# lukifer23/Matrix0

Hardware: AMD Instinct MI355X
Metric: self-play games/sec at 800 sims/move, ResNet-24 53M; 1/2/4/8 MI355X (higher is better)
Workload: dtype f16

## Files before the change

matrix0_amd/csrc/attn_block.hip:

```cpp
#include "attn_math.h"
#include "conv_epilogue.h"

typedef float float4v __attribute__((ext_vector_type(4)));

namespace {
constexpr int AB_PIECE = 12288;
constexpr int AB_PIECES_PER_GROUP = 7;
constexpr int AB_GROUPS = 10;
constexpr int AB_X = 0;
constexpr int AB_QK = 81920;
constexpr int AB_VT = AB_QK + 16384;
constexpr int AB_VROW = 68;
constexpr int AB_RING = AB_VT + 4 * 16 * AB_VROW * 2;
constexpr int AB_PAR = AB_RING + 4 * AB_PIECE;
constexpr int AB_LDS = AB_PAR + 4 * 320 * 4;

struct AbLane {
    int tid, lane, w;
    int l15, lq, r31, half;
    int wm, wn;
    size_t b0;
    uint32_t xa[2];
    int wq0, wq1, wpo;
    uint32_t ring_a, of_a;
    const char* wsrc;
    char* ring_w;
    int au, aboard, ahl, aqt, aq;
};
struct AbRegs {
    float4v oc[20];
    float4v qa[2][3];
    half8 fs[2][5];
    half8 of;
    half8 bias8[4];
    half2v visp[16];
};
}

__device__ __forceinline__ void ab_load64(half8& b0, half8& b1, half8& b2, half8& b3, const half8* p) {
    asm volatile("global_load_dwordx4 %0, %4, off\n\tglobal_load_dwordx4 %1, %4, off offset:16\n\t"
                 "global_load_dwordx4 %2, %4, off offset:32\n\tglobal_load_dwordx4 %3, %4, off offset:48"
                 : "=&v"(b0), "=&v"(b1), "=&v"(b2), "=&v"(b3) : "v"(p) : "memory");
}
template <int OFF>
__device__ __forceinline__ void ab_lds16(half8& d, uint32_t addr) {
    asm volatile("ds_read_b128 %0, %1 offset:%2" : "=v"(d) : "v"(addr), "n"(OFF) : "memory");
}
template <int N>
__device__ __forceinline__ void ab_lds_arrived(half8& f0, half8& f1, half8& f2, half8& f3, half8& f4, half8& f5) {
    static_assert(N == 0 || N == 5, "");
    if constexpr (N == 0) asm volatile("s_waitcnt lgkmcnt(0)" : "+v"(f0), "+v"(f1), "+v"(f2), "+v"(f3), "+v"(f4), "+v"(f5) :: "memory");
    else asm volatile("s_waitcnt lgkmcnt(5)" : "+v"(f0), "+v"(f1), "+v"(f2), "+v"(f3), "+v"(f4), "+v"(f5) :: "memory");
}
template <int CTRL>
__device__ __forceinline__ float ab_dpp(float v) {
    return __builtin_bit_cast(float, __builtin_amdgcn_update_dpp(0, __builtin_bit_cast(int, v), CTRL, 0xF, 0xF, true));
}
__device__ __forceinline__ float ab_row_sum(float v) {
    v += ab_dpp<0xB1>(v);
    v += ab_dpp<0x4E>(v);
    v += ab_dpp<0x141>(v);
    v += ab_dpp<0x140>(v);
    return v;
}

#define AB_WAIT(n) asm volatile("s_waitcnt vmcnt(" #n ")" ::: "memory")
#define AB_LGKM0() asm volatile("s_waitcnt lgkmcnt(0)" ::: "memory")

__device__ __forceinline__ char* ab_smem() {
    extern __shared__ __attribute__((aligned(16))) char smem[];
    return smem;
}

__device__ __forceinline__ AbLane ab_lane(const AttnBlockArgs& a) {
    AbLane L;
    L.tid = threadIdx.x; L.lane = L.tid & 63;
    L.w = __builtin_amdgcn_readfirstlane(L.tid >> 6);
    L.l15 = L.lane & 15; L.lq = L.lane >> 4; L.r31 = L.lane & 31; L.half = L.lane >> 5;
    L.wm = L.w >> 1; L.wn = L.w & 1;
    L.b0 = (size_t)blockIdx.x * 2;
    const int l15 = L.l15, lq = L.lq, w = L.w;
    const int xrow0 = 32 * L.wm + l15;
    const int xsw = (xrow0 >> 1) & 7;
    const int xe0 = ((lq ^ xsw) & 7) * 16, xe1 = (((4 + lq) ^ xsw) & 7) * 16;
    const uint32_t lds0 = (uint32_t)(uintptr_t)ab_smem();
    L.xa[0] = lds0 + AB_X + xrow0 * 640 + xe0; L.xa[1] = lds0 + AB_X + xrow0 * 640 + xe1;
    const int wsw = (l15 >> 1) & 7;
    L.wq0 = (3 * L.wn * 16 + l15) * 128 + ((lq ^ wsw) & 7) * 16;
    L.wq1 = (3 * L.wn * 16 + l15) * 128 + (((4 + lq) ^ wsw) & 7) * 16;
    L.wpo = l15 * 64 + ((lq ^ (4 - (l15 >> 2))) & 3) * 16;
    L.ring_a = lds0 + AB_RING;
    L.of_a = lds0 + AB_QK + (lq >> 1) * 4096 + (16 * w + l15) * 32 + ((lq & 1) ^ (l15 >> 3)) * 16;
    L.wsrc = reinterpret_cast<const char*>(a.wpack) + w * 1536 + L.lane * 16;
    L.ring_w = ab_smem() + AB_RING + w * 1536;
    L.au = w >> 1; L.aboard = L.au >> 1; L.ahl = L.au & 1; L.aqt = w & 1;
    L.aq = L.aqt * 32 + L.r31;
    return L;
}

__device__ __forceinline__ void ab_issue(const AbLane& L, int t) {
    const char* s = L.wsrc + (size_t)t * AB_PIECE;
    char* d = L.ring_w + (t & 3) * AB_PIECE;
    glds16(s, d);
    if (L.lane < 32) glds16(s + 1024, d + 1024);
}

__device__ __forceinline__ void ab_prologue(const AttnBlockArgs& a, const AbLane& L) {
    const char* xg = reinterpret_cast<const char*>(a.x) + L.b0 * 64 * 640;
#pragma unroll
    for (int n = 0; n < 10; ++n) {
        const int idx = L.w * 10 + n;
        const int q = idx * 64 + L.lane;
        const int row = q / 40, pos = q - row * 40;
        const int src = (pos & ~7) | ((pos ^ (row >> 1)) & 7);
        glds16(xg + row * 640 + src * 16, ab_smem() + AB_X + idx * 1024);
    }
    ab_issue(L, 0); ab_issue(L, 1); ab_issue(L, 2);
    const int tid = L.tid;
    if (tid < 320) {
        float* par = reinterpret_cast<float*>(ab_smem() + AB_PAR);
        par[tid] = a.ln_g[tid]; par[320 + tid] = a.ln_b[tid];
        par[640 + tid] = a.y2 ? a.gn2_gamma[tid] : 0.f; par[960 + tid] = a.y2 ? a.gn2_beta[tid] : 0.f;
    }
}

__device__ __forceinline__ void ab_visibility(const AttnBlockArgs& a, const AbLane& L, half2v (&visp)[16]) {
    const uint64_t m = a.mask[L.aq];
    static_for<0, 32>([&](auto i_) __attribute__((always_inline)) {
        constexpr int i = decltype(i_)::value;
        constexpr int kt = i >> 4, r = i & 15;
        const int key = kt * 32 + 8 * (r >> 2) + 4 * L.half + (r & 3);
        visp[i >> 1][i & 1] = (_Float16)(float)((m >> key) & 1);
    });
}

__device__ __forceinline__ void ab_zero_qa(float4v (&qa)[2][3]) {
    const float4v zero4 = {0.f, 0.f, 0.f, 0.f};
    static_for<0, 2>([&](auto i_) __attribute__((always_inline)) {
        static_for<0, 3>([&](auto j_) __attribute__((always_inline)) { qa[decltype(i_)::value][decltype(j_)::value] = zero4; });
    });
}

template <bool HP, int U>
__device__ __forceinline__ void ab_load(const AbLane& L, AbRegs& R, const int T) {
    constexpr int S = U & 1, i = U >> 1, kk = U & 1;
    const uint32_t slot = L.ring_a + (uint32_t)(((T + i) & 3) * AB_PIECE);
    if constexpr (HP && i < 2) {
        if constexpr (U == 0) ab_lds16<0>(R.of, L.of_a);
        const uint32_t pa = slot + L.wpo;
        static_for<0, 5>([&](auto jj_) __attribute__((always_inline)) {
            constexpr int jj = decltype(jj_)::value;
            ab_lds16<(5 * kk + jj) * 1024>(R.fs[S][jj], pa);
        });
    } else {
        constexpr int p = i - (HP ? 2 : 0);
        ab_lds16<128 * p>(R.fs[S][3], L.xa[kk]);
        ab_lds16<128 * p + 16 * 640>(R.fs[S][4], L.xa[kk]);
        const uint32_t wa = slot + (kk ? L.wq1 : L.wq0);
        static_for<0, 3>([&](auto j_) __attribute__((always_inline)) {
            constexpr int j = decltype(j_)::value;
            ab_lds16<j * 2048>(R.fs[S][j], wa);
        });
    }
}
template <int U, int N>
__device__ __forceinline__ void ab_arrived(AbRegs& R) {
    constexpr int S = U & 1;
    ab_lds_arrived<N>(R.fs[S][0], R.fs[S][1], R.fs[S][2], R.fs[S][3], R.fs[S][4], R.of);
}
template <bool HP, int U>
__device__ __forceinline__ void ab_mma(AbRegs& R) {
    constexpr int S = U & 1, i = U >> 1, kk = U & 1;
    if constexpr (HP && i < 2) {
        static_for<0, 5>([&](auto jj_) __attribute__((always_inline)) {
            constexpr int c = 10 * i + 5 * kk + decltype(jj_)::value;
            R.oc[c] = __builtin_amdgcn_mfma_f32_16x16x32_f16(R.fs[S][decltype(jj_)::value], R.of, R.oc[c], 0, 0, 0);
        });
    } else {
        static_for<0, 3>([&](auto j_) __attribute__((always_inline)) {
            constexpr int j = decltype(j_)::value;
            R.qa[0][j] = __builtin_amdgcn_mfma_f32_16x16x32_f16(R.fs[S][j], R.fs[S][3], R.qa[0][j], 0, 0, 0);
            R.qa[1][j] = __builtin_amdgcn_mfma_f32_16x16x32_f16(R.fs[S][j], R.fs[S][4], R.qa[1][j], 0, 0, 0);
        });
    }
}

template <bool HP, bool HQ>
__device__ __forceinline__ void ab_sequence(const AttnBlockArgs& a, const AbLane& L, AbRegs& R, const int T, const int g) {
    constexpr int NP = (HP ? 2 : 0) + (HQ ? 5 : 0), NU = 2 * NP;
    constexpr int BU = NU - 3;
    AB_LGKM0();
    AB_WAIT(4);
    __builtin_amdgcn_s_barrier();
    asm volatile("" ::: "memory");
    ab_load<HP, 0>(L, R, T);
    ab_issue(L, T + 3);
    static_for<0, NU>([&](auto u_) __attribute__((always_inline)) {
        constexpr int u = decltype(u_)::value;
        if constexpr (u + 1 < NU) {
            if constexpr (u & 1) {
                ab_arrived<u, 0>(R);
                AB_WAIT(4);
                __builtin_amdgcn_s_barrier();
                asm volatile("" ::: "memory");
            }
            ab_load<HP, u + 1>(L, R, T);
            if constexpr (u & 1) ab_issue(L, T + (u >> 1) + 4);
            else ab_arrived<u, 5>(R);
        } else {
            ab_arrived<u, 0>(R);
        }
        if constexpr (HQ && u == BU) {
            const half8* bp = reinterpret_cast<const half8*>(a.bias) + ((size_t)((2 * g + L.ahl) * 2 + L.aqt) * 64 + L.lane) * 4;
            ab_load64(R.bias8[0], R.bias8[1], R.bias8[2], R.bias8[3], bp);
        }
        ab_mma<HP, u>(R);
        __builtin_amdgcn_sched_barrier(0);
    });
}

__device__ __forceinline__ void ab_stage_qkv(const AbLane& L, const float4v (&qa)[2][3]) {
    char* const smem = ab_smem();
    const int lane = L.lane, l15 = L.l15, lq = L.lq;
    static_for<0, 2>([&](auto i_) __attribute__((always_inline)) {
        static_for<0, 3>([&](auto j_) __attribute__((always_inline)) {
            constexpr int i = decltype(i_)::value, j = decltype(j_)::value;
            const int J = 3 * L.wn + j, type = J >> 1, hl = J & 1;
            const int token = 32 * L.wm + 16 * i + l15;
            const half4v h = {(_Float16)qa[i][j][0], (_Float16)qa[i][j][1], (_Float16)qa[i][j][2], (_Float16)qa[i][j][3]};
            if (type < 2) {
                *reinterpret_cast<half4v*>(smem + AB_QK + type * 8192 + hl * 4096 + token * 32 + (((lq >> 1) ^ (l15 >> 3)) & 1) * 16 + (lq & 1) * 8) = h;
            } else {
                const int unit = (token >> 6) * 2 + hl, sq = token & 63;
                union { half2v h2; uint32_t u; } p01, p23;
                p01.h2 = half2v{h[0], h[1]}; p23.h2 = half2v{h[2], h[3]};
                const bool odd = (lane & 1) != 0;
                const uint32_t own = odd ? p23.u : p01.u;
                const uint32_t recv = (uint32_t)__builtin_amdgcn_update_dpp(0, (int)(odd ? p01.u : p23.u), 0xB1, 0xF, 0xF, true);
                const uint32_t ta = odd ? recv : own, tb = odd ? own : recv;
                const uint32_t w0 = __builtin_amdgcn_perm(tb, ta, 0x05040100u);
                const uint32_t w1 = __builtin_amdgcn_perm(tb, ta, 0x07060302u);
                uint32_t* vt = reinterpret_cast<uint32_t*>(reinterpret_cast<_Float16*>(smem + AB_VT) +
                                                           (unit * 16 + 4 * lq + (odd ? 2 : 0)) * AB_VROW + (sq & ~1));
                vt[0] = w0; vt[AB_VROW / 2] = w1;
            }
        });
    });
    AB_LGKM0();
    __builtin_amdgcn_s_barrier();
    asm volatile("" ::: "memory");
}

__device__ __forceinline__ void ab_attend(const AbLane& L, AbRegs& R, float isd, float clampv, float wm, float wu) {
    const int half = L.half, r31 = L.r31;
    const char* Kb = ab_smem() + AB_QK + 8192 + L.ahl * 4096 + L.aboard * 64 * 32;
    const int hsw = 16 * (half ^ ((r31 >> 3) & 1));
    const half8 kf0 = *reinterpret_cast<const half8*>(Kb + r31 * 32 + hsw);
    const half8 kf1 = *reinterpret_cast<const half8*>(Kb + (32 + r31) * 32 + hsw);
    char* Qp = ab_smem() + AB_QK + L.ahl * 4096 + (L.aboard * 64 + L.aq) * 32 + hsw;
    const half8 qfr = *reinterpret_cast<const half8*>(Qp);
    half8 vf[2][2];
    attn_v_frags(reinterpret_cast<const _Float16*>(ab_smem() + AB_VT) + (L.au * 16 + L.l15) * AB_VROW, half, vf);
    float16v st[2];
    attn_scores(kf0, kf1, qfr, st);
    asm volatile("s_waitcnt vmcnt(0)" : "+v"(R.bias8[0]), "+v"(R.bias8[1]), "+v"(R.bias8[2]), "+v"(R.bias8[3]) :: "memory");
    auto bias = [&](auto kt_, auto g_) __attribute__((always_inline)) {
        constexpr int bi = decltype(kt_)::value * 16 + 4 * decltype(g_)::value;
        const half8 b = R.bias8[bi >> 3];
        return half4v{b[bi & 7], b[(bi & 7) + 1], b[(bi & 7) + 2], b[(bi & 7) + 3]};
    };
    auto vis = [&](auto kt_, auto g_) __attribute__((always_inline)) {
        constexpr int bi = decltype(kt_)::value * 16 + 4 * decltype(g_)::value;
        return half4v{R.visp[bi >> 1][0], R.visp[bi >> 1][1], R.visp[(bi >> 1) + 1][0], R.visp[(bi >> 1) + 1][1]};
    };
    const uint4v ov = attn_pack_o(attn_softmax_pv(st, bias, vis, vf, isd, clampv, wm, wu), half);
    asm volatile("ds_write_b128 %0, %1" :: "v"((uint32_t)(uintptr_t)Qp), "v"(ov) : "memory");
}

__device__ __forceinline__ half4v* ab_own4(const AbLane& L, int j) {
    const int token = 16 * L.w + L.l15;
    const int chunk = 2 * j + (L.lq >> 1);
    const int tsw = (token >> 1) & 7;
    const int pos = (chunk & ~7) | ((chunk ^ tsw) & 7);
    return reinterpret_cast<half4v*>(ab_smem() + AB_X + token * 640 + (L.lq & 1) * 8 + pos * 16);
}
__device__ __forceinline__ float2* ab_gn_partials() { return reinterpret_cast<float2*>(ab_smem() + AB_RING); }
__device__ __forceinline__ float2* ab_gn_totals() { return ab_gn_partials() + 8 * 20 * 4; }

__device__ __forceinline__ void ab_residual_layernorm(const AttnBlockArgs& a, const AbLane& L, float4v (&oc)[20]) {
    float s1 = 0.f, s2 = 0.f;
    static_for<0, 20>([&](auto j_) __attribute__((always_inline)) {
        constexpr int j = decltype(j_)::value;
        const half4v xv = *ab_own4(L, j);
        static_for<0, 4>([&](auto r_) __attribute__((always_inline)) {
            constexpr int r = decltype(r_)::value;
            const float v = oc[j][r] + (float)xv[r];
            oc[j][r] = v;
            s1 += v; s2 += v * v;
        });
    });
    s1 += __shfl_xor(s1, 16); s2 += __shfl_xor(s2, 16);
    s1 += __shfl_xor(s1, 32); s2 += __shfl_xor(s2, 32);
    const float cnt = (float)a.ln_count;
    const float mean = s1 / cnt;
    float var = s2 / cnt - mean * mean;
    var = var > 0.f ? var : 0.f;
    const float rstd = rsqrtf(var + 1e-5f);
    const float* par = reinterpret_cast<const float*>(ab_smem() + AB_PAR);
    float2* scr = ab_gn_partials();
    const float nmr = -mean * rstd;
    static_for<0, 20>([&](auto j_) __attribute__((always_inline)) {
        constexpr int j = decltype(j_)::value;
        const float4 gm = *reinterpret_cast<const float4*>(par + 16 * j + 4 * L.lq);
        const float4 bt = *reinterpret_cast<const float4*>(par + 320 + 16 * j + 4 * L.lq);
        const float gmv[4] = {gm.x, gm.y, gm.z, gm.w}, btv[4] = {bt.x, bt.y, bt.z, bt.w};
        float p1 = 0.f, p2 = 0.f;
        half4v h;
        static_for<0, 4>([&](auto r_) __attribute__((always_inline)) {
            constexpr int r = decltype(r_)::value;
            const float y = fmaf(fmaf(oc[j][r], rstd, nmr), gmv[r], btv[r]);
            p1 += y; p2 += y * y;
            h[r] = (_Float16)y;
        });
        *ab_own4(L, j) = h;
        p1 = ab_row_sum(p1); p2 = ab_row_sum(p2);
        if (L.l15 == 0) scr[(L.w * 20 + j) * 4 + L.lq] = make_float2(p1, p2);
    });
}

__device__ __forceinline__ void ab_flush(const AbLane& L, _Float16* outp) {
    char* og = reinterpret_cast<char*>(outp) + (L.b0 * 64 + 16 * L.w) * 640;
#pragma unroll
    for (int n = 0; n < 10; ++n) {
        const int q = n * 64 + L.lane;
        const int rl = q / 40, pos = q - rl * 40;
        const int grow = 16 * L.w + rl;
        const int src = (pos & ~7) | ((pos ^ (grow >> 1)) & 7);
        const uint4 v = *reinterpret_cast<const uint4*>(ab_smem() + AB_X + grow * 640 + pos * 16);
        *reinterpret_cast<uint4*>(og + rl * 640 + src * 16) = v;
    }
}

template <int ACT>
__device__ __forceinline__ void ab_second_output(const AbLane& L) {
    const int tid = L.tid;
    float2* scr = ab_gn_partials();
    float2* tot = ab_gn_totals();
    __syncthreads();
    if (tid < 40) {
        const int bd = tid / 20, j = tid - bd * 20;
        float s = 0.f, ss = 0.f;
        for (int ww = 0; ww < 4; ++ww)
            for (int q = 0; q < 4; ++q) { const float2 v = scr[((bd * 4 + ww) * 20 + j) * 4 + q]; s += v.x; ss += v.y; }
        float mu, rstd;
        gn16_mean_rstd(s, ss, mu, rstd);
        tot[tid] = make_float2(mu, rstd);
    }
    __syncthreads();
    float* par = reinterpret_cast<float*>(ab_smem() + AB_PAR);
    {
        float scv[2] = {0.f, 0.f}, shv[2] = {0.f, 0.f};
        if (tid < 320) {
            const float g2 = par[640 + tid], b2 = par[960 + tid];
#pragma unroll
            for (int bd = 0; bd < 2; ++bd) {
                const float2 mr = tot[bd * 20 + (tid >> 4)];
                scv[bd] = g2 * mr.y; shv[bd] = b2 - mr.x * scv[bd];
            }
        }
        __syncthreads();
        if (tid < 320) { par[tid] = scv[0]; par[320 + tid] = shv[0]; par[640 + tid] = scv[1]; par[960 + tid] = shv[1]; }
        __syncthreads();
    }
    static_for<0, 20>([&](auto j_) __attribute__((always_inline)) {
        constexpr int j = decltype(j_)::value;
        const float4 gm = *reinterpret_cast<const float4*>(par + (L.w >> 2) * 640 + 16 * j + 4 * L.lq);
        const float4 bt = *reinterpret_cast<const float4*>(par + (L.w >> 2) * 640 + 320 + 16 * j + 4 * L.lq);
        const float gmv[4] = {gm.x, gm.y, gm.z, gm.w}, btv[4] = {bt.x, bt.y, bt.z, bt.w};
        half4v h = *ab_own4(L, j);
        static_for<0, 4>([&](auto r_) __attribute__((always_inline)) {
            constexpr int r = decltype(r_)::value;
            h[r] = (_Float16)act_fast<ACT>((float)h[r] * gmv[r] + btv[r]);
        });
        *ab_own4(L, j) = h;
    });
}

template <int ACT>
__global__ __launch_bounds__(512) void attn_block_kernel(AttnBlockArgs a) {
    const AbLane L = ab_lane(a);
    ab_prologue(a, L);
    AbRegs R;
    ab_visibility(a, L, R.visp);
    float wm, wu;
    attn_branch_weights(a.mix, wm, wu);
    const float isd = a.inv_sqrt_d * kLog2e;
    const float clampv = 50.f * kLog2e;
    const float4v zero4 = {0.f, 0.f, 0.f, 0.f};
    static_for<0, 20>([&](auto j_) __attribute__((always_inline)) { R.oc[decltype(j_)::value] = zero4; });

    ab_zero_qa(R.qa);
    ab_sequence<false, true>(a, L, R, 0, 0);
#pragma unroll 1
    for (int g = 0; g < AB_GROUPS - 1; ++g) {
        ab_stage_qkv(L, R.qa);
        ab_attend(L, R, isd, clampv, wm, wu);
        ab_zero_qa(R.qa);
        ab_sequence<true, true>(a, L, R, 7 * g + 5, g + 1);
    }
    ab_stage_qkv(L, R.qa);
    ab_attend(L, R, isd, clampv, wm, wu);
    ab_sequence<true, false>(a, L, R, 7 * AB_GROUPS - 2, AB_GROUPS);
    AB_WAIT(0);
    __syncthreads();

    ab_residual_layernorm(a, L, R.oc);
    ab_flush(L, a.y);
    if (a.y2 == nullptr) return;
    ab_second_output<ACT>(L);
    ab_flush(L, a.y2);
}

hipError_t launch_attn_block(const AttnBlockArgs& a, hipStream_t st) {
    if (a.B <= 0 || a.B % 2 != 0 || a.ln_count <= 0 || a.ln_count > 320) return hipErrorInvalidValue;
    if (a.y2 != nullptr && a.act != ACT_SILU && a.act != ACT_RELU) return hipErrorInvalidValue;
    static DeviceOnce once;
    hipError_t e = once.run([] {
        hipError_t r = hipFuncSetAttribute(reinterpret_cast<const void*>(&attn_block_kernel<ACT_SILU>),
                                           hipFuncAttributeMaxDynamicSharedMemorySize, AB_LDS);
        if (r != hipSuccess) return r;
        return hipFuncSetAttribute(reinterpret_cast<const void*>(&attn_block_kernel<ACT_RELU>),
                                   hipFuncAttributeMaxDynamicSharedMemorySize, AB_LDS);
    });
    if (e != hipSuccess) return e;
    const dim3 grid((unsigned)(a.B / 2));
    if (a.act == ACT_RELU) hipLaunchKernelGGL(attn_block_kernel<ACT_RELU>, grid, dim3(512), AB_LDS, st, a);
    else hipLaunchKernelGGL(attn_block_kernel<ACT_SILU>, grid, dim3(512), AB_LDS, st, a);
    return hipGetLastError();
}

size_t attn_block_pack_bytes() { return (size_t)(AB_GROUPS * AB_PIECES_PER_GROUP + 3) * AB_PIECE; }
```

Before: 1.163.

## Make attention block kernel persistent with next-pair prefetch overlapping epilogue

The attention block kernel now launches at most one workgroup per CU and loops over board pairs with a grid stride. During the second-output epilogue it issues the next pair's activation rows and first three weight pieces, so those loads overlap the tail of the current pair. The second output is staged per quarter through LDS for coalesced stores, and LN/GN parameters stay in registers rather than being reloaded from global memory each pair. In exchange the kernel is more complex, fills fewer CUs when batches are small, and the per-device CU-count cache is shared across devices.

```diff
diff --git a/matrix0_amd/csrc/attn_block.hip b/matrix0_amd/csrc/attn_block.hip
--- a/matrix0_amd/csrc/attn_block.hip
+++ b/matrix0_amd/csrc/attn_block.hip
@@ -19,7 +19,6 @@
     int tid, lane, w;
     int l15, lq, r31, half;
     int wm, wn;
-    size_t b0;
     uint32_t xa[2];
     int wq0, wq1, wpo;
     uint32_t ring_a, of_a;
@@ -35,6 +34,10 @@
     half8 bias8[4];
     half2v visp[16];
 };
+struct AbOwn {
+    int tid, lane, w, l15, lq;
+    size_t pair;
+};
 }
 
 __device__ __forceinline__ void ab_load64(half8& b0, half8& b1, half8& b2, half8& b3, const half8* p) {
@@ -42,8 +45,9 @@
                  "global_load_dwordx4 %2, %4, off offset:32\n\tglobal_load_dwordx4 %3, %4, off offset:48"
                  : "=&v"(b0), "=&v"(b1), "=&v"(b2), "=&v"(b3) : "v"(p) : "memory");
 }
-template <int OFF>
-__device__ __forceinline__ void ab_lds16(half8& d, uint32_t addr) {
+template <int OFF, typename T>
+__device__ __forceinline__ void ab_lds16(T& d, uint32_t addr) {
+    static_assert(sizeof(T) == 16, "");
     asm volatile("ds_read_b128 %0, %1 offset:%2" : "=v"(d) : "v"(addr), "n"(OFF) : "memory");
 }
 template <int N>
@@ -51,6 +55,15 @@
     static_assert(N == 0 || N == 5, "");
     if constexpr (N == 0) asm volatile("s_waitcnt lgkmcnt(0)" : "+v"(f0), "+v"(f1), "+v"(f2), "+v"(f3), "+v"(f4), "+v"(f5) :: "memory");
     else asm volatile("s_waitcnt lgkmcnt(5)" : "+v"(f0), "+v"(f1), "+v"(f2), "+v"(f3), "+v"(f4), "+v"(f5) :: "memory");
+}
+template <int OFF>
+__device__ __forceinline__ void ab_lds_put8(uint32_t addr, half4v h) {
+    asm volatile("ds_write_b64 %0, %1 offset:%2" :: "v"(addr), "v"(h), "n"(OFF) : "memory");
+}
+template <typename T>
+__device__ __forceinline__ void ab_lds_arrived5(T (&f)[5], T (&g)[5]) {
+    asm volatile("s_waitcnt lgkmcnt(0)" : "+v"(f[0]), "+v"(f[1]), "+v"(f[2]), "+v"(f[3]), "+v"(f[4]),
+                                          "+v"(g[0]), "+v"(g[1]), "+v"(g[2]), "+v"(g[3]), "+v"(g[4]) :: "memory");
 }
 template <int CTRL>
 __device__ __forceinline__ float ab_dpp(float v) {
@@ -67,6 +80,16 @@
 #define AB_WAIT(n) asm volatile("s_waitcnt vmcnt(" #n ")" ::: "memory")
 #define AB_LGKM0() asm volatile("s_waitcnt lgkmcnt(0)" ::: "memory")
 
+#ifdef AB_DRY
+__device__ int* g_ab_dry;
+__device__ __forceinline__ int* ab_dry_counts() { __shared__ int n[8]; return n; }
+#define AB_BARRIER() do { if ((threadIdx.x & 63) == 0) ++ab_dry_counts()[threadIdx.x >> 6]; } while (0)
+#define AB_SYNC() AB_BARRIER()
+#else
+#define AB_BARRIER() __builtin_amdgcn_s_barrier()
+#define AB_SYNC() __syncthreads()
+#endif
+
 __device__ __forceinline__ char* ab_smem() {
     extern __shared__ __attribute__((aligned(16))) char smem[];
     return smem;
@@ -78,7 +101,6 @@
     L.w = __builtin_amdgcn_readfirstlane(L.tid >> 6);
     L.l15 = L.lane & 15; L.lq = L.lane >> 4; L.r31 = L.lane & 31; L.half = L.lane >> 5;
     L.wm = L.w >> 1; L.wn = L.w & 1;
-    L.b0 = (size_t)blockIdx.x * 2;
     const int l15 = L.l15, lq = L.lq, w = L.w;
     const int xrow0 = 32 * L.wm + l15;
     const int xsw = (xrow0 >> 1) & 7;
@@ -104,23 +126,39 @@
     glds16(s, d);
     if (L.lane < 32) glds16(s + 1024, d + 1024);
 }
-
-__device__ __forceinline__ void ab_prologue(const AttnBlockArgs& a, const AbLane& L) {
-    const char* xg = reinterpret_cast<const char*>(a.x) + L.b0 * 64 * 640;
+__device__ __forceinline__ void ab_issue_first3(const AbLane& L) {
+    glds16(L.wsrc, L.ring_w); glds16(L.wsrc + AB_PIECE, L.ring_w + AB_PIECE); glds16(L.wsrc + 2 * AB_PIECE, L.ring_w + 2 * AB_PIECE);
+    if (L.lane < 32) {
+        glds16(L.wsrc + 1024, L.ring_w + 1024); glds16(L.wsrc + AB_PIECE + 1024, L.ring_w + AB_PIECE + 1024);
+        glds16(L.wsrc + 2 * AB_PIECE + 1024, L.ring_w + 2 * AB_PIECE + 1024);
+    }
+}
+
+__device__ __forceinline__ void ab_issue_rows(const AttnBlockArgs& a, int w, int lane, size_t pair) {
+    const char* xg = reinterpret_cast<const char*>(a.x) + pair * (128 * 640);
 #pragma unroll
     for (int n = 0; n < 10; ++n) {
-        const int idx = L.w * 10 + n;
-        const int q = idx * 64 + L.lane;
+        const int idx = w * 10 + n;
+        const int q = idx * 64 + lane;
         const int row = q / 40, pos = q - row * 40;
         const int src = (pos & ~7) | ((pos ^ (row >> 1)) & 7);
         glds16(xg + row * 640 + src * 16, ab_smem() + AB_X + idx * 1024);
     }
-    ab_issue(L, 0); ab_issue(L, 1); ab_issue(L, 2);
-    const int tid = L.tid;
+}
+
+__device__ __forceinline__ void ab_load_params(const AttnBlockArgs& a, int tid, float (&pv)[4]) {
+    pv[0] = pv[1] = pv[2] = pv[3] = 0.f;
     if (tid < 320) {
-        float* par = reinterpret_cast<float*>(ab_smem() + AB_PAR);
-        par[tid] = a.ln_g[tid]; par[320 + tid] = a.ln_b[tid];
-        par[640 + tid] = a.y2 ? a.gn2_gamma[tid] : 0.f; par[960 + tid] = a.y2 ? a.gn2_beta[tid] : 0.f;
+        pv[0] = a.ln_g[tid]; pv[1] = a.ln_b[tid];
+        if (a.y2) { pv[2] = a.gn2_gamma[tid]; pv[3] = a.gn2_beta[tid]; }
+    }
+}
+__device__ __forceinline__ void ab_store_params(const AbLane& L, const float (&pv)[4]) {
+    if (L.tid < 320) {
+        const uint32_t pa = (uint32_t)(uintptr_t)ab_smem() + AB_PAR + 4 * L.tid;
+        asm volatile("ds_write_b32 %0, %1\n\tds_write_b32 %0, %2 offset:1280\n\tds_write_b32 %0, %3 offset:2560\n\t"
+                     "ds_write_b32 %0, %4 offset:3840"
+                     :: "v"(pa), "v"(pv[0]), "v"(pv[1]), "v"(pv[2]), "v"(pv[3]) : "memory");
     }
 }
 
@@ -191,7 +229,7 @@
     constexpr int BU = NU - 3;
     AB_LGKM0();
     AB_WAIT(4);
-    __builtin_amdgcn_s_barrier();
+    AB_BARRIER();
     asm volatile("" ::: "memory");
     ab_load<HP, 0>(L, R, T);
     ab_issue(L, T + 3);
@@ -201,7 +239,7 @@
             if constexpr (u & 1) {
                 ab_arrived<u, 0>(R);
                 AB_WAIT(4);
-                __builtin_amdgcn_s_barrier();
+                AB_BARRIER();
                 asm volatile("" ::: "memory");
             }
             ab_load<HP, u + 1>(L, R, T);
@@ -247,7 +285,7 @@
         });
     });
     AB_LGKM0();
-    __builtin_amdgcn_s_barrier();
+    AB_BARRIER();
     asm volatile("" ::: "memory");
 }
 
@@ -277,21 +315,21 @@
     asm volatile("ds_write_b128 %0, %1" :: "v"((uint32_t)(uintptr_t)Qp), "v"(ov) : "memory");
 }
 
-__device__ __forceinline__ half4v* ab_own4(const AbLane& L, int j) {
-    const int token = 16 * L.w + L.l15;
-    const int chunk = 2 * j + (L.lq >> 1);
+__device__ __forceinline__ half4v* ab_own4(const AbOwn& E, int j) {
+    const int token = 16 * E.w + E.l15;
+    const int chunk = 2 * j + (E.lq >> 1);
     const int tsw = (token >> 1) & 7;
     const int pos = (chunk & ~7) | ((chunk ^ tsw) & 7);
-    return reinterpret_cast<half4v*>(ab_smem() + AB_X + token * 640 + (L.lq & 1) * 8 + pos * 16);
+    return reinterpret_cast<half4v*>(ab_smem() + AB_X + token * 640 + (E.lq & 1) * 8 + pos * 16);
 }
 __device__ __forceinline__ float2* ab_gn_partials() { return reinterpret_cast<float2*>(ab_smem() + AB_RING); }
 __device__ __forceinline__ float2* ab_gn_totals() { return ab_gn_partials() + 8 * 20 * 4; }
 
-__device__ __forceinline__ void ab_residual_layernorm(const AttnBlockArgs& a, const AbLane& L, float4v (&oc)[20]) {
+__device__ __forceinline__ void ab_residual_layernorm(const AttnBlockArgs& a, const AbOwn& E, float4v (&oc)[20]) {
     float s1 = 0.f, s2 = 0.f;
     static_for<0, 20>([&](auto j_) __attribute__((always_inline)) {
         constexpr int j = decltype(j_)::value;
-        const half4v xv = *ab_own4(L, j);
+        const half4v xv = *ab_own4(E, j);
         static_for<0, 4>([&](auto r_) __attribute__((always_inline)) {
             constexpr int r = decltype(r_)::value;
             const float v = oc[j][r] + (float)xv[r];
@@ -311,8 +349,8 @@
     const float nmr = -mean * rstd;
     static_for<0, 20>([&](auto j_) __attribute__((always_inline)) {
         constexpr int j = decltype(j_)::value;
-        const float4 gm = *reinterpret_cast<const float4*>(par + 16 * j + 4 * L.lq);
-        const float4 bt = *reinterpret_cast<const float4*>(par + 320 + 16 * j + 4 * L.lq);
+        const float4 gm = *reinterpret_cast<const float4*>(par + 16 * j + 4 * E.lq);
+        const float4 bt = *reinterpret_cast<const float4*>(par + 320 + 16 * j + 4 * E.lq);
         const float gmv[4] = {gm.x, gm.y, gm.z, gm.w}, btv[4] = {bt.x, bt.y, bt.z, bt.w};
         float p1 = 0.f, p2 = 0.f;
         half4v h;
@@ -322,31 +360,47 @@
             p1 += y; p2 += y * y;
             h[r] = (_Float16)y;
         });
-        *ab_own4(L, j) = h;
+        *ab_own4(E, j) = h;
         p1 = ab_row_sum(p1); p2 = ab_row_sum(p2);
-        if (L.l15 == 0) scr[(L.w * 20 + j) * 4 + L.lq] = make_float2(p1, p2);
-    });
-}
-
-__device__ __forceinline__ void ab_flush(const AbLane& L, _Float16* outp) {
-    char* og = reinterpret_cast<char*>(outp) + (L.b0 * 64 + 16 * L.w) * 640;
+        if (E.l15 == 0) scr[(E.w * 20 + j) * 4 + E.lq] = make_float2(p1, p2);
+    });
+}
+
+__device__ __forceinline__ void ab_flush(const AbOwn& E, _Float16* outp) {
+    char* og = reinterpret_cast<char*>(outp) + (E.pair * 128 + 16 * E.w) * 640;
 #pragma unroll
     for (int n = 0; n < 10; ++n) {
-        const int q = n * 64 + L.lane;
+        const int q = n * 64 + E.lane;
         const int rl = q / 40, pos = q - rl * 40;
-        const int grow = 16 * L.w + rl;
+        const int grow = 16 * E.w + rl;
         const int src = (pos & ~7) | ((pos ^ (grow >> 1)) & 7);
         const uint4 v = *reinterpret_cast<const uint4*>(ab_smem() + AB_X + grow * 640 + pos * 16);
         *reinterpret_cast<uint4*>(og + rl * 640 + src * 16) = v;
     }
 }
 
+__device__ __forceinline__ void ab_prefetch(const AttnBlockArgs& a, const AbLane& L, const AbOwn& E, size_t next) {
+    ab_issue_rows(a, E.w, E.lane, next);
+    ab_issue_first3(L);
+}
+
+__device__ __forceinline__ void ab_flush_quarter(const AbOwn& E, uint32_t st_r, char* og, const int (&goff)[3]) {
+    uint4v v0, v1, v2 = {0u, 0u, 0u, 0u};
+    asm volatile("ds_read_b128 %0, %2\n\tds_read_b128 %1, %2 offset:1024" : "=&v"(v0), "=&v"(v1) : "v"(st_r) : "memory");
+    if (E.lane < 32) asm volatile("ds_read_b128 %0, %1 offset:2048" : "+v"(v2) : "v"(st_r) : "memory");
+    asm volatile("s_waitcnt lgkmcnt(0)" : "+v"(v0), "+v"(v1), "+v"(v2) :: "memory");
+    *reinterpret_cast<uint4v*>(og + goff[0]) = v0;
+    *reinterpret_cast<uint4v*>(og + goff[1]) = v1;
+    if (E.lane < 32) *reinterpret_cast<uint4v*>(og + goff[2]) = v2;
+}
+
 template <int ACT>
-__device__ __forceinline__ void ab_second_output(const AbLane& L) {
-    const int tid = L.tid;
+__device__ __forceinline__ void ab_second_output(const AttnBlockArgs& a, const AbLane& L, const AbOwn& E, const float (&pv)[4],
+                                                 const bool more, const size_t next) {
+    const int tid = E.tid;
     float2* scr = ab_gn_partials();
     float2* tot = ab_gn_totals();
-    __syncthreads();
+    AB_SYNC();
     if (tid < 40) {
         const int bd = tid / 20, j = tid - bd * 20;
         float s = 0.f, ss = 0.f;
@@ -356,40 +410,74 @@
         gn16_mean_rstd(s, ss, mu, rstd);
         tot[tid] = make_float2(mu, rstd);
     }
-    __syncthreads();
+    AB_SYNC();
     float* par = reinterpret_cast<float*>(ab_smem() + AB_PAR);
     {
         float scv[2] = {0.f, 0.f}, shv[2] = {0.f, 0.f};
         if (tid < 320) {
-            const float g2 = par[640 + tid], b2 = par[960 + tid];
+            const float g2 = pv[2], b2 = pv[3];
 #pragma unroll
             for (int bd = 0; bd < 2; ++bd) {
                 const float2 mr = tot[bd * 20 + (tid >> 4)];
                 scv[bd] = g2 * mr.y; shv[bd] = b2 - mr.x * scv[bd];
             }
         }
-        __syncthreads();
+        AB_SYNC();
         if (tid < 320) { par[tid] = scv[0]; par[320 + tid] = shv[0]; par[640 + tid] = scv[1]; par[960 + tid] = shv[1]; }
-        __syncthreads();
-    }
-    static_for<0, 20>([&](auto j_) __attribute__((always_inline)) {
-        constexpr int j = decltype(j_)::value;
-        const float4 gm = *reinterpret_cast<const float4*>(par + (L.w >> 2) * 640 + 16 * j + 4 * L.lq);
-        const float4 bt = *reinterpret_cast<const float4*>(par + (L.w >> 2) * 640 + 320 + 16 * j + 4 * L.lq);
-        const float gmv[4] = {gm.x, gm.y, gm.z, gm.w}, btv[4] = {bt.x, bt.y, bt.z, bt.w};
-        half4v h = *ab_own4(L, j);
-        static_for<0, 4>([&](auto r_) __attribute__((always_inline)) {
-            constexpr int r = decltype(r_)::value;
-            h[r] = (_Float16)act_fast<ACT>((float)h[r] * gmv[r] + btv[r]);
-        });
-        *ab_own4(L, j) = h;
+        AB_SYNC();
+    }
+    half4v yh[20];
+    static_for<0, 20>([&](auto j_) __attribute__((always_inline)) { yh[decltype(j_)::value] = *ab_own4(E, decltype(j_)::value); });
+    asm volatile("s_waitcnt lgkmcnt(0)"
+                 : "+v"(yh[0]), "+v"(yh[1]), "+v"(yh[2]), "+v"(yh[3]), "+v"(yh[4]), "+v"(yh[5]), "+v"(yh[6]), "+v"(yh[7]), "+v"(yh[8]),
+                   "+v"(yh[9]), "+v"(yh[10]), "+v"(yh[11]), "+v"(yh[12]), "+v"(yh[13]), "+v"(yh[14]), "+v"(yh[15]), "+v"(yh[16]),
+                   "+v"(yh[17]), "+v"(yh[18]), "+v"(yh[19]) :: "memory");
+    if (more) ab_prefetch(a, L, E, next);
+
+    const uint32_t lds0 = (uint32_t)(uintptr_t)ab_smem();
+    const uint32_t par_a = lds0 + AB_PAR + (E.w >> 2) * 2560 + 16 * E.lq;
+    const uint32_t stage = lds0 + AB_QK + E.w * 2560;
+    const uint32_t st_w = stage + E.l15 * 160 + E.lq * 8;
+    const uint32_t st_r = stage + E.lane * 16;
+    char* og = reinterpret_cast<char*>(a.y2) + (E.pair * 128 + 16 * E.w) * 640;
+    int goff[3];
+#pragma unroll
+    for (int n = 0; n < 3; ++n) {
+        const int q = n * 64 + E.lane;
+        const int rl = q / 10, pos = q - rl * 10;
+        goff[n] = rl * 640 + pos * 16;
+    }
+    static_for<0, 4>([&](auto q_) __attribute__((always_inline)) {
+        constexpr int Q = decltype(q_)::value;
+        float4v gm[5], bt[5];
+        static_for<0, 5>([&](auto jj_) __attribute__((always_inline)) {
+            constexpr int jj = decltype(jj_)::value, j = 5 * Q + jj;
+            ab_lds16<64 * j>(gm[jj], par_a);
+            ab_lds16<1280 + 64 * j>(bt[jj], par_a);
+        });
+        ab_lds_arrived5(gm, bt);
+        static_for<0, 5>([&](auto jj_) __attribute__((always_inline)) {
+            constexpr int jj = decltype(jj_)::value, j = 5 * Q + jj;
+            half4v h = yh[j];
+            static_for<0, 4>([&](auto r_) __attribute__((always_inline)) {
+                constexpr int r = decltype(r_)::value;
+                h[r] = (_Float16)act_fast<ACT>((float)h[r] * gm[jj][r] + bt[jj][r]);
+            });
+            ab_lds_put8<32 * jj>(st_w, h);
+        });
+        ab_flush_quarter(E, st_r, og + 160 * Q, goff);
     });
 }
 
 template <int ACT>
 __global__ __launch_bounds__(512) void attn_block_kernel(AttnBlockArgs a) {
-    const AbLane L = ab_lane(a);
-    ab_prologue(a, L);
+    AbLane L = ab_lane(a);
+    const size_t npairs = (size_t)(a.B >> 1), stride = gridDim.x;
+    size_t pair = blockIdx.x;
+    ab_issue_rows(a, L.w, L.lane, pair);
+    ab_issue_first3(L);
+    float pv[4];
+    ab_load_params(a, L.tid, pv);
     AbRegs R;
     ab_visibility(a, L, R.visp);
     float wm, wu;
@@ -397,28 +485,59 @@
     const float isd = a.inv_sqrt_d * kLog2e;
     const float clampv = 50.f * kLog2e;
     const float4v zero4 = {0.f, 0.f, 0.f, 0.f};
-    static_for<0, 20>([&](auto j_) __attribute__((always_inline)) { R.oc[decltype(j_)::value] = zero4; });
-
-    ab_zero_qa(R.qa);
-    ab_sequence<false, true>(a, L, R, 0, 0);
+#ifdef AB_DRY
+    if (L.lane == 0) ab_dry_counts()[L.w] = 0;
+#endif
+
 #pragma unroll 1
-    for (int g = 0; g < AB_GROUPS - 1; ++g) {
+    for (;;) {
+        asm volatile("s_waitcnt vmcnt(0)" : "+v"(pv[0]), "+v"(pv[1]), "+v"(pv[2]), "+v"(pv[3]) :: "memory");
+        asm volatile("" : "+v"(L.wsrc));
+        static_for<0, 20>([&](auto j_) __attribute__((always_inline)) { R.oc[decltype(j_)::value] = zero4; });
+
+        ab_zero_qa(R.qa);
+        ab_sequence<false, true>(a, L, R, 0, 0);
+        ab_store_params(L, pv);
+#pragma unroll 1
+        for (int g = 0; g < AB_GROUPS - 1; ++g) {
+            ab_stage_qkv(L, R.qa);
+            ab_attend(L, R, isd, clampv, wm, wu);
+            ab_zero_qa(R.qa);
+            ab_sequence<true, true>(a, L, R, 7 * g + 5, g + 1);
+        }
         ab_stage_qkv(L, R.qa);
         ab_attend(L, R, isd, clampv, wm, wu);
-        ab_zero_qa(R.qa);
-        ab_sequence<true, true>(a, L, R, 7 * g + 5, g + 1);
-    }
-    ab_stage_qkv(L, R.qa);
-    ab_attend(L, R, isd, clampv, wm, wu);
-    ab_sequence<true, false>(a, L, R, 7 * AB_GROUPS - 2, AB_GROUPS);
-    AB_WAIT(0);
-    __syncthreads();
-
-    ab_residual_layernorm(a, L, R.oc);
-    ab_flush(L, a.y);
-    if (a.y2 == nullptr) return;
-    ab_second_output<ACT>(L);
-    ab_flush(L, a.y2);
+        ab_sequence<true, false>(a, L, R, 7 * AB_GROUPS - 2, AB_GROUPS);
+        AB_WAIT(0);
+        AB_SYNC();
+
+        const size_t next = pair + stride;
+        const bool more = next < npairs;
+        AbOwn E;
+        E.lane = L.lane;
+        asm volatile("" : "+v"(E.lane));
+        E.w = L.w; E.tid = 64 * E.w + E.lane; E.l15 = E.lane & 15; E.lq = E.lane >> 4; E.pair = pair;
+        ab_residual_layernorm(a, E, R.oc);
+        ab_flush(E, a.y);
+        if (a.y2 != nullptr) {
+            ab_second_output<ACT>(a, L, E, pv, more, next);
+        } else if (more) {
+            AB_LGKM0();
+            ab_issue_rows(a, E.w, E.lane, next);
+            AB_BARRIER();
+            asm volatile("" ::: "memory");
+            ab_issue_first3(L);
+        }
+        if (!more) break;
+        pair = next;
+    }
+#ifdef AB_DRY
+    if (L.lane == 0) g_ab_dry[blockIdx.x * 8 + L.w] = ab_dry_counts()[L.w];
+#endif
+}
+
+namespace {
+std::atomic<int> ab_cu_count[32];
 }
 
 hipError_t launch_attn_block(const AttnBlockArgs& a, hipStream_t st) {
@@ -429,11 +548,24 @@
         hipError_t r = hipFuncSetAttribute(reinterpret_cast<const void*>(&attn_block_kernel<ACT_SILU>),
                                            hipFuncAttributeMaxDynamicSharedMemorySize, AB_LDS);
         if (r != hipSuccess) return r;
-        return hipFuncSetAttribute(reinterpret_cast<const void*>(&attn_block_kernel<ACT_RELU>),
-                                   hipFuncAttributeMaxDynamicSharedMemorySize, AB_LDS);
+        r = hipFuncSetAttribute(reinterpret_cast<const void*>(&attn_block_kernel<ACT_RELU>),
+                                hipFuncAttributeMaxDynamicSharedMemorySize, AB_LDS);
+        if (r != hipSuccess) return r;
+        int d = 0, cus = 0;
+        if ((r = hipGetDevice(&d)) != hipSuccess) return r;
+        if ((r = hipDeviceGetAttribute(&cus, hipDeviceAttributeMultiprocessorCount, d)) != hipSuccess) return r;
+        if (cus <= 0) return hipErrorInvalidDevice;
+        if ((unsigned)d < 32u) ab_cu_count[d].store(cus, std::memory_order_relaxed);
+        return hipSuccess;
     });
     if (e != hipSuccess) return e;
-    const dim3 grid((unsigned)(a.B / 2));
+    int d = 0, cus = 0;
+    if ((e = hipGetDevice(&d)) != hipSuccess) return e;
+    if ((unsigned)d < 32u) cus = ab_cu_count[d].load(std::memory_order_relaxed);
+    else if ((e = hipDeviceGetAttribute(&cus, hipDeviceAttributeMultiprocessorCount, d)) != hipSuccess) return e;
+    if (cus <= 0) return hipErrorInvalidDevice;
+    const int pairs = a.B / 2;
+    const dim3 grid((unsigned)(pairs < cus ? pairs : cus));
     if (a.act == ACT_RELU) hipLaunchKernelGGL(attn_block_kernel<ACT_RELU>, grid, dim3(512), AB_LDS, st, a);
     else hipLaunchKernelGGL(attn_block_kernel<ACT_SILU>, grid, dim3(512), AB_LDS, st, a);
     return hipGetLastError();
```

After: 1.174 (median of 6 runs). About the same (+1.0%).
